# mit-han-lab/qserve

Hardware: AMD Instinct MI355X
Metric: decode tokens/sec/GPU Llama-3-8B W4A8KV4 bs=64 (higher is better)
Workload: dtype int8xint4->int32 (MFMA) + fp16; 1 GPU; Llama-3-8B W4A8 per-channel KV4 decode step, bs=64, context 1024->+512 (BASELINE.json configs[1]); global_batch=64, context_start=1030, parallelism=tp1, hipgraph=True, layers=32, launches_per_layer=8

## Files before the change

qserve_amd/csrc/attention_mfma.hip:

```cpp
#include "attn_host.h"
#include "kv_quant.h"
#include <mutex>
#include <string.h>

namespace {

constexpr int PAGE_TOK = 64;
constexpr int DH = 128;
constexpr int DHB = 64;
constexpr int UT = 32;
constexpr int USB = UT * DHB;
constexpr int NW = attn_plan::DECODE_WAVES_KV4;
constexpr int NWT = NW;
constexpr int QS_ATTNQ_CAP = 4096;
constexpr int QS_ATTNQ_ROW = 4096;
constexpr int SVC = NW - 1;
#ifndef QS_SEQ
#define QS_SEQ(x) asm volatile("" : "+v"(x))
#endif
constexpr int MAXP = 192;

typedef __attribute__((address_space(1))) uint8_t* g_u8;
typedef __attribute__((address_space(1))) uint16_t* g_u16;
__device__ __forceinline__ void wave_quant_store4(_Float16 v0, _Float16 v1, uint8_t* dst_, __half* scale_p_,
                                                  __half* zero_p_, int lane) {
    g_u8 dst = (g_u8)dst_;
    g_u16 scale_p = (g_u16)reinterpret_cast<uint16_t*>(scale_p_), zero_p = (g_u16)reinterpret_cast<uint16_t*>(zero_p_);
    const float mx = wave_max_dpp(fmaxf((float)v0, (float)v1));
    const float mn = wave_min_dpp(fminf((float)v0, (float)v1));
    const QParams p = make_qparams<true>(mn, mx);
    const unsigned u0 = quant_u8(v0, p), u1 = quant_u8(v1, p);
    dst[lane] = (uint8_t)((u0 & 0xFu) | (u1 << 4));
    if (lane == 0) {
        *scale_p = __builtin_bit_cast(uint16_t, p.scale);
        *zero_p = __builtin_bit_cast(uint16_t, p.zero);
    }
}

__device__ __forceinline__ u32 and_or(u32 x, u32 m, u32 c) {
    return (x & m) | c;
}

typedef __attribute__((address_space(3))) const uint8_t* lds_u8;

template <int G, int EXP = 0>
__global__ __launch_bounds__(NWT * 64, 4) void decode_attention_mfma_kernel(
    const _Float16* __restrict__ q, const _Float16* __restrict__ k, const _Float16* __restrict__ v,
    const int64_t* __restrict__ kv_pointers, const int* __restrict__ lengths, _Float16* __restrict__ out,
    int num_heads, int num_kv_heads, int64_t q_stride0, int64_t kv_stride0, int max_blocks, int timestep,
    float rope_base, const float2* __restrict__ rope_tab, int rope_tab_len, int nsplit, float* __restrict__ ws,
    int8_t* __restrict__ qout, __half* __restrict__ qscale, __half* __restrict__ qrowsum, unsigned* __restrict__ qcounters,
    int kflags) {
    constexpr bool PROFILE = (EXP & 64) != 0;
    __shared__ __attribute__((aligned(16))) uint8_t s_kv[2 * NW * 2 * USB];
    __shared__ __attribute__((aligned(16))) _Float16 s_meta[NW][2][4][UT];
    __shared__ __attribute__((aligned(16))) _Float16 s_q[G][DH];
    __shared__ __attribute__((aligned(16))) _Float16 s_qp[16][DH];
    __shared__ __attribute__((aligned(16))) _Float16 s_knew[DH];
    __shared__ __attribute__((aligned(16))) _Float16 s_vnew[DH];
    __shared__ float s_cur[16];
    __shared__ float2 s_qc[16];
    __shared__ float s_m[NW][G], s_l[NW][G];
    __shared__ int s_flag;

    const int tid = threadIdx.x, lane = tid & 63;
    const int wave = __builtin_amdgcn_readfirstlane(tid >> 6);
    const int hkv = blockIdx.x, b = blockIdx.y;
    __shared__ unsigned long long s_stamps[(EXP & 32) ? NWT * 16 : 1];
    auto stamp = [&](int i) {
        if constexpr (EXP & 32) {
            const unsigned long long t = __builtin_amdgcn_s_memtime();
            if (lane == 0) s_stamps[wave * 16 + i] = t;
        }
    };
    if constexpr (EXP & 32) {
        if (lane < 16) s_stamps[wave * 16 + lane] = 0;
    }
    stamp(0);
    if (!(kflags & 2)) {
        const u32 fa = (u32)(uintptr_t)(__attribute__((address_space(3))) void*)(&s_flag);
        if (tid == SVC * 64) asm volatile("ds_write_b32 %0, %1" ::"v"(fa), "v"(0));
        asm volatile("s_waitcnt lgkmcnt(0)\n\ts_barrier");
    }
    const _Float16* qb = q + (size_t)b * q_stride0 + (size_t)hkv * G * DH;
    const _Float16* kb = k + (size_t)b * kv_stride0 + (size_t)hkv * DH;
    const _Float16* vb = v + (size_t)b * kv_stride0 + (size_t)hkv * DH;
    auto uni_ptr = [](const void* x) -> uint64_t {
        return ((uint64_t)(u32)__builtin_amdgcn_readfirstlane((u32)((uint64_t)(uintptr_t)x >> 32)) << 32) |
               (uint64_t)(u32)__builtin_amdgcn_readfirstlane((u32)(uint64_t)(uintptr_t)x);
    };
    const uint64_t qb_s = uni_ptr(qb), kb_s = uni_ptr(kb), vb_s = uni_ptr(vb);
    const int64_t* ktab = kv_pointers + (size_t)b * 2 * max_blocks;
    const int64_t* vtab = ktab + max_blocks;
    const bool spec = (nsplit == 1 || blockIdx.z == 0);
    if (wave == SVC) {
        asm volatile("s_setprio 3");
        if constexpr (!(EXP & 4)) {
            const u32 lane4 = (u32)lane * 4u;
            auto glds4 = [&](uint64_t sb, const _Float16* dst) {
                const u32 ld = __builtin_amdgcn_readfirstlane((u32)(uintptr_t)(__attribute__((address_space(3))) const void*)dst);
                asm volatile("s_mov_b32 m0, %2\n\ts_nop 4\n\tglobal_load_lds_dword %0, %1" ::"v"(lane4), "s"(sb), "s"(ld) : "memory");
            };
#pragma unroll
            for (int h = 0; h < G; ++h) glds4(qb_s + (uint64_t)(h * DH * 2), &s_q[h][0]);
            glds4(kb_s, &s_knew[0]);
            glds4(vb_s, &s_vnew[0]);
        }
        stamp(5);
    }
    int64_t kpage0, vpage0, kpage7, vpage7;
    int len_raw, gen_raw;
    {
        const int p0 = (wave >> 1) < max_blocks ? (wave >> 1) : 0, p7 = ((wave + NW - 1) >> 1) < max_blocks ? ((wave + NW - 1) >> 1) : 0;
        const uint64_t a0 = uni_ptr(ktab + p0), a1 = uni_ptr(vtab + p0), a2 = uni_ptr(ktab + p7), a3 = uni_ptr(vtab + p7);
        const uint64_t a4 = uni_ptr(lengths ? (const void*)(lengths + b) : (const void*)ktab);
        const uint64_t a5 = uni_ptr(qcounters ? (const void*)(qcounters + b) : (const void*)ktab);
        asm volatile("s_load_dwordx2 %0, %6, 0x0\n\ts_load_dwordx2 %1, %7, 0x0\n\ts_load_dwordx2 %2, %8, 0x0\n\t"
                     "s_load_dwordx2 %3, %9, 0x0\n\ts_load_dword %4, %10, 0x0\n\ts_load_dword %5, %11, 0x0\n\ts_waitcnt lgkmcnt(0)"
                     : "=&s"(kpage0), "=&s"(vpage0), "=&s"(kpage7), "=&s"(vpage7), "=&s"(len_raw), "=&s"(gen_raw)
                     : "s"(a0), "s"(a1), "s"(a2), "s"(a3), "s"(a4), "s"(a5)
                     : "memory");
    }
    const int tl = lengths ? len_raw - 1 : timestep;
    if (tl < 0) return;
    stamp(1);
    const float inv_sqrt = 0.08838834764831845f;
    const float qk_scale = inv_sqrt * 1.4426950408889634f;
    constexpr int GP = G <= 4 ? 4 : 8;
    const int li = lane & 15, tg = lane >> 4;
    uint8_t* const s_kw = s_kv + wave * (2 * USB);
    uint8_t* const s_vw = s_kv + (NW + wave) * (2 * USB);

    const int nunits = (tl + UT - 1) >> 5;
    const int z = blockIdx.z;
    const int ups = (nunits + nsplit - 1) / nsplit;
    const int u_begin = z * ups, u_end = min(nunits, u_begin + ups);
    typedef const __attribute__((address_space(1))) void* gptr_t;
    typedef __attribute__((address_space(3))) void* lptr_t;
    auto next_pages = [&](int p, int64_t& kn, int64_t& vn) {
        const uint64_t ka = (uint64_t)(uintptr_t)(ktab + p), va = (uint64_t)(uintptr_t)(vtab + p);
        const uint64_t ks = ((uint64_t)(u32)__builtin_amdgcn_readfirstlane((u32)(ka >> 32)) << 32) |
                            (uint64_t)(u32)__builtin_amdgcn_readfirstlane((u32)ka);
        const uint64_t vs = ((uint64_t)(u32)__builtin_amdgcn_readfirstlane((u32)(va >> 32)) << 32) |
                            (uint64_t)(u32)__builtin_amdgcn_readfirstlane((u32)va);
        asm volatile("s_load_dwordx2 %0, %2, 0x0\n\ts_load_dwordx2 %1, %3, 0x0\n\ts_waitcnt lgkmcnt(0)"
                     : "=&s"(kn), "=&s"(vn) : "s"(ks), "s"(vs) : "memory");
    };
    auto uni64 = [&](int64_t x) -> uint64_t {
        return ((uint64_t)(u32)__builtin_amdgcn_readfirstlane((u32)((uint64_t)x >> 32)) << 32) |
               (uint64_t)(u32)__builtin_amdgcn_readfirstlane((u32)(uint64_t)x);
    };
    auto glds16 = [&](uint64_t sbase, u32 voff, u32 ldst) {
        if constexpr (!(EXP & 1))
            asm volatile("s_mov_b32 m0, %2\n\ts_nop 4\n\tglobal_load_lds_dwordx4 %0, %1 nt" ::"v"(voff), "s"(sbase), "s"(ldst) : "memory");
        else
            asm volatile("s_mov_b32 m0, %2\n\ts_nop 4\n\tglobal_load_lds_dwordx4 %0, %1" ::"v"(voff), "s"(sbase), "s"(ldst) : "memory");
    };
    auto glds4_lower = [&](uint64_t sbase, u32 voff, u32 ldst) {
        uint64_t ex;
        asm volatile("s_mov_b64 %0, exec\n\ts_mov_b32 exec_hi, 0\n\ts_mov_b32 m0, %3\n\ts_nop 4\n\tglobal_load_lds_dword %1, %2\n\ts_mov_b64 exec, %0"
                     : "=&s"(ex) : "v"(voff), "s"(sbase), "s"(ldst) : "memory");
    };
    auto glds4_upper = [&](uint64_t sbase, u32 voff, u32 ldst) {
        uint64_t ex;
        asm volatile("s_mov_b64 %0, exec\n\ts_mov_b32 exec_lo, 0\n\ts_mov_b32 m0, %3\n\ts_nop 4\n\tglobal_load_lds_dword %1, %2\n\ts_mov_b64 exec, %0"
                     : "=&s"(ex) : "v"(voff), "s"(sbase), "s"(ldst) : "memory");
    };
    const u32 meta_lane = (u32)(((lane >> 4) & 1) * num_kv_heads * PAGE_TOK * 2 + (lane & 15) * 4);
    const u32 lane16 = (u32)lane * 16u;
    const u32 lds_k = __builtin_amdgcn_readfirstlane((u32)(uintptr_t)(lptr_t)s_kw);
    const u32 lds_v = __builtin_amdgcn_readfirstlane((u32)(uintptr_t)(lptr_t)s_vw);
    const u32 lds_m = __builtin_amdgcn_readfirstlane((u32)(uintptr_t)(lptr_t)(&s_meta[wave][0][0][0]));
    const u32 meta_off = (u32)(num_kv_heads * PAGE_TOK * DHB + hkv * PAGE_TOK * 2);
    const u32 data_off = (u32)(hkv * PAGE_TOK * DHB);
    auto dma_data = [&](uint64_t base, u32 ldst, int valid_tok) {
        if (valid_tok >= UT) {
            glds16(base, lane16, ldst);
            glds16(base + 1024, lane16, ldst + 1024);
        } else {
            if ((lane >> 2) < valid_tok || lane == 0) glds16(base, lane16, ldst);
            if (16 + (lane >> 2) < valid_tok || lane == 0) glds16(base + 1024, lane16, ldst + 1024);
        }
    };
    auto dma_a = [&](int64_t page, int half, int slot, int valid_tok) {
        const uint64_t pg = uni64(page);
        glds4_lower(pg + (meta_off + (u32)(half * UT * 2)), meta_lane, lds_m + (u32)(slot * (4 * UT * 2)));
        dma_data(pg + (data_off + (u32)(half * USB)), lds_k + (u32)(slot * USB), valid_tok);
    };
    auto dma_b = [&](int64_t page, int half, int slot, int valid_tok) {
        const uint64_t pg = uni64(page);
        glds4_upper(pg + (meta_off + (u32)(half * UT * 2)), meta_lane, lds_m + (u32)(slot * (4 * UT * 2)));
        dma_data(pg + (data_off + (u32)(half * USB)), lds_v + (u32)(slot * USB), valid_tok);
    };
    const int blk = tl >> 6, slot_new = tl & 63;
    const int nu = max(u_end - u_begin, 0);
    const bool svc_free = (nu + NW - 2) / (NW - 1) == (nu + NW - 1) / NW;
    const int PS = svc_free ? NW - 1 : NW;
    const int u_first = u_begin + wave;
    auto unit_of = [&](int i) -> int { return u_first + i * PS; };
    const int cnt = ((!svc_free || wave != SVC) && wave < nu) ? (nu - wave + PS - 1) / PS : 0;
    const bool spec2 = spec && PS == NW - 1;
    const bool use_flag = !(kflags & 2);
    auto first_round = [&](int which) {
        if (cnt > 0) {
            const int u1 = unit_of(1);
            int64_t kfirst = kpage0, vfirst = vpage0, ksecond = kpage7, vsecond = vpage7;
            if ((which & 1) && !spec) next_pages(u_first >> 1, kfirst, vfirst);
            if ((which & 2) && cnt > 1 && !spec2) next_pages(u1 >> 1, ksecond, vsecond);
            if (which & 1) {
                const int vt0 = min(UT, tl - u_first * UT);
                dma_a(kfirst, u_first & 1, 0, vt0);
                stamp(3);
                dma_b(vfirst, u_first & 1, 0, vt0);
            }
            if ((which & 2) && cnt > 1) {
                const int vt1 = min(UT, tl - u1 * UT);
                dma_a(ksecond, u1 & 1, 1, vt1);
                dma_b(vsecond, u1 & 1, 1, vt1);
            }
        }
        if (which & 2) stamp(2);
    };
    auto new_token_work = [&]() {
        if (z == 0) {
            uint8_t* pgk = reinterpret_cast<uint8_t*>(ktab[blk]);
            __half* sck = reinterpret_cast<__half*>(pgk + (size_t)num_kv_heads * PAGE_TOK * DHB);
            wave_quant_store4(s_knew[2 * lane], s_knew[2 * lane + 1], pgk + ((size_t)hkv * PAGE_TOK + slot_new) * DHB,
                              sck + hkv * PAGE_TOK + slot_new, sck + num_kv_heads * PAGE_TOK + hkv * PAGE_TOK + slot_new, lane);
            uint8_t* pgv = reinterpret_cast<uint8_t*>(vtab[blk]);
// ... 70 lines not shown
                so = xor32(xor16(so));
                if (tg == 0) s_qc[li] = make_float2(se + 16.f * so, 1024.f * (se + so));
            }
            if (use_flag) {
                asm volatile("s_waitcnt lgkmcnt(0)" ::: "memory");
                if (lane == 0) *(volatile __attribute__((address_space(3))) int*)(&s_flag) = 1;
            } else {
                asm volatile("s_waitcnt lgkmcnt(0)\n\ts_barrier" ::: "memory");
            }
            asm volatile("s_setprio 0");
            stamp(4);
            if (svc_free) new_token_work();
        } else {
            if (use_flag) {
                asm volatile("s_waitcnt lgkmcnt(0)" ::: "memory");
                if (lane == 0) *(volatile __attribute__((address_space(3))) int*)(&s_flag) = 1;
            } else {
                asm volatile("s_waitcnt lgkmcnt(0)\n\ts_barrier" ::: "memory");
            }
        }
        first_round(3);
    }

    const float2 qc = s_qc[li & (GP - 1)];
    const float qsum = qc.x, nqoff = -qc.y;
    if constexpr (EXP & 32) {
        float probe = nqoff;
        asm volatile("" : "+v"(probe));
        stamp(11);
    }

    u32 c_lo = 0x000F000Fu, c_hi = 0x00F000F0u, c_magic = 0x64006400u;
    asm volatile("" : "+v"(c_lo), "+v"(c_hi), "+v"(c_magic));

    v4f acc[8];
#pragma unroll
    for (int e = 0; e < 8; ++e) acc[e] = (v4f){0.f, 0.f, 0.f, 0.f};
    float m_run = -3.0e38f, l_part = 0.f, corr = 0.f, psum = 0.f;

    constexpr int NS = GP == 4 ? 2 : 4;
    const int tok0 = 16 * (li >> 3) + 4 * tg + (GP == 4 ? 2 * ((li >> 2) & 1) : 0);
    u32 kl0 = (u32)(uintptr_t)(lptr_t)s_kw + (u32)(li * DHB + 16 * tg);
    u32 vl0 = (u32)(uintptr_t)(lptr_t)s_vw + (u32)((4 * tg) * DHB + 4 * li);
    u32 ml0 = (u32)(uintptr_t)(lptr_t)(&s_meta[wave][0][0][0]) + (u32)(2 * tok0);
    asm volatile("" : "+v"(kl0), "+v"(vl0), "+v"(ml0));
    h8 qB[4];
    {
        const lds_u8 ql = (lds_u8)(&s_qp[0][0]) + (li * (DH * 2) + 64 * tg);
#pragma unroll
        for (int w = 0; w < 4; ++w) qB[w] = *(const __attribute__((address_space(3))) h8*)(ql + 16 * w);
    }

    int it = 0;
    int rem = cnt - 1;
    for (int u = u_first; it < cnt; ++it, --rem, u = unit_of(it)) {
        const bool has2 = rem >= 2;
        asm volatile("; QS_LOOP_BEGIN\n\ts_cmp_eq_u32 %0, 0\n\ts_cbranch_scc1 1f\n\ts_waitcnt vmcnt(9)\n\ts_branch 2f\n1:\n\ts_waitcnt vmcnt(3)\n2:"
                     ::"s"(rem) : "memory", "scc");
        if (it < 2) stamp(5 + 2 * it);
        const int slot = it & 1;
        const int valid = min(UT, tl - u * UT);
        const bool full = valid == UT;
        const int u2 = unit_of(it + 2), valid2 = min(UT, tl - u2 * UT);
        int64_t kpage_next = 0, vpage_next = 0;
        if (has2) next_pages(u2 >> 1, kpage_next, vpage_next);
        if constexpr (EXP & 2) {
            if (has2) dma_a(kpage_next, u2 & 1, slot, valid2);
            asm volatile("s_cmp_lt_u32 %0, 2\n\ts_cbranch_scc1 1f\n\ts_waitcnt vmcnt(9)\n\ts_branch 3f\n1:\n\ts_cmp_eq_u32 %0, 0\n\ts_cbranch_scc1 2f\n\t"
                         "s_waitcnt vmcnt(6)\n\ts_branch 3f\n2:\n\ts_waitcnt vmcnt(0)\n3:" ::"s"(rem) : "memory", "scc");
            if (has2) dma_b(vpage_next, u2 & 1, slot, valid2);
            continue;
        }
        const lds_u8 kl = (lds_u8)(kl0 + (u32)(slot * USB));
        const lds_u8 vl = (lds_u8)(vl0 + (u32)(slot * USB));
        const lds_u8 ml = (lds_u8)(ml0 + (u32)(slot * (4 * UT * 2)));
        v4f craw[2];
#pragma unroll
        for (int t = 0; t < 2; ++t) {
            const v4u raw = *(const __attribute__((address_space(3))) v4u*)(kl + 16 * t * DHB);
            v4f c = {nqoff, nqoff, nqoff, nqoff};
#pragma unroll
            for (int w = 0; w < 4; ++w) {
                const u32 x = raw[w], xs = x >> 8;
                const v4u a4 = {and_or(x, c_lo, c_magic), and_or(x, c_hi, c_magic), and_or(xs, c_lo, c_magic),
                                and_or(xs, c_hi, c_magic)};
                c = __builtin_amdgcn_mfma_f32_16x16x32_f16(__builtin_bit_cast(h8, a4), qB[w], c, 0, 0, 0);
            }
            craw[t] = c;
        }
        float sc[NS];
        float m_new;
        {
            float ksf[NS], kzf[NS];
            if constexpr (GP == 4) {
                const h2 ks = *(const __attribute__((address_space(3))) h2*)(ml);
                const h2 kz = *(const __attribute__((address_space(3))) h2*)(ml + UT * 2);
                ksf[0] = (float)ks[0], ksf[1] = (float)ks[1], kzf[0] = (float)kz[0], kzf[1] = (float)kz[1];
            } else {
                const h4 ks = *(const __attribute__((address_space(3))) h4*)(ml);
                const h4 kz = *(const __attribute__((address_space(3))) h4*)(ml + UT * 2);
#pragma unroll
                for (int j = 0; j < 4; ++j) ksf[j] = (float)ks[j], kzf[j] = (float)kz[j];
            }
#pragma unroll
            for (int j = 0; j < NS; ++j) {
                int x;
                if constexpr (GP == 4) {
                    const float c00 = craw[0][j], c02 = craw[0][2 + j], c10 = craw[1][j], c12 = craw[1][2 + j];
                    x = __builtin_bit_cast(int, c00);
                    x = __builtin_amdgcn_update_dpp(x, __builtin_bit_cast(int, c02), 0x114, 0xF, 0x2, false);
                    x = __builtin_amdgcn_update_dpp(x, __builtin_bit_cast(int, c10), 0x118, 0xF, 0x4, false);
                    x = __builtin_amdgcn_update_dpp(x, __builtin_bit_cast(int, c12), 0x11C, 0xF, 0x8, false);
                } else {
                    const float c0 = craw[0][j], c1 = craw[1][j];
                    x = __builtin_amdgcn_update_dpp(__builtin_bit_cast(int, c0), __builtin_bit_cast(int, c1), 0x118, 0xF, 0xC, false);
                }
                sc[j] = (ksf[j] * qk_scale) * (__builtin_bit_cast(float, x) - kzf[j] * qsum);
            }
            if (!full) {
#pragma unroll
                for (int j = 0; j < NS; ++j)
                    if (tok0 + j >= valid) sc[j] = -3.0e38f;
            }
            asm volatile("s_waitcnt lgkmcnt(0)" ::: "memory");
            if (has2) dma_a(kpage_next, u2 & 1, slot, valid2);
            float mx = sc[0];
#pragma unroll
            for (int j = 1; j < NS; ++j) mx = fmaxf(mx, sc[j]);
            if constexpr (GP == 4) asm volatile("s_nop 1\n\tv_max_f32_dpp %0, %0, %0 row_ror:4 row_mask:0xf bank_mask:0xf" : "+v"(mx));
            asm volatile("s_nop 1\n\tv_max_f32_dpp %0, %0, %0 row_ror:8 row_mask:0xf bank_mask:0xf" : "+v"(mx));
            {
                const int xi = __builtin_bit_cast(int, mx);
                const auto r = __builtin_amdgcn_permlane16_swap(xi, xi, false, false);
                mx = fmaxf(__builtin_bit_cast(float, (int)r[0]), __builtin_bit_cast(float, (int)r[1]));
            }
            {
                const int xi = __builtin_bit_cast(int, mx);
                const auto r = __builtin_amdgcn_permlane32_swap(xi, xi, false, false);
                mx = fmaxf(__builtin_bit_cast(float, (int)r[0]), __builtin_bit_cast(float, (int)r[1]));
            }
            m_new = fmaxf(m_run, mx);
            const float alpha = __builtin_amdgcn_exp2f(m_run - m_new);
            m_run = m_new;
            if (__any(alpha != 1.0f)) {
                l_part *= alpha;
                corr *= alpha;
                psum *= alpha;
#pragma unroll
                for (int e = 0; e < 8; ++e) acc[e] *= alpha;
            }
        }
        asm volatile("s_cmp_lt_u32 %0, 2\n\ts_cbranch_scc1 1f\n\ts_waitcnt vmcnt(9)\n\ts_branch 3f\n1:\n\ts_cmp_eq_u32 %0, 0\n\ts_cbranch_scc1 2f\n\t"
                     "s_waitcnt vmcnt(6)\n\ts_branch 3f\n2:\n\ts_waitcnt vmcnt(0)\n3:" ::"s"(rem) : "memory", "scc");
        u32 pbv[4];
        {
            float vsf[NS], vzf[NS];
            if constexpr (GP == 4) {
                const h2 vs = *(const __attribute__((address_space(3))) h2*)(ml + 2 * UT * 2);
                const h2 vz = *(const __attribute__((address_space(3))) h2*)(ml + 3 * UT * 2);
                vsf[0] = (float)vs[0], vsf[1] = (float)vs[1], vzf[0] = (float)vz[0], vzf[1] = (float)vz[1];
            } else {
                const h4 vs = *(const __attribute__((address_space(3))) h4*)(ml + 2 * UT * 2);
                const h4 vz = *(const __attribute__((address_space(3))) h4*)(ml + 3 * UT * 2);
#pragma unroll
                for (int j = 0; j < 4; ++j) vsf[j] = (float)vs[j], vzf[j] = (float)vz[j];
            }
            float pp[NS];
#pragma unroll
            for (int j = 0; j < NS; ++j) {
                const float pe = __builtin_amdgcn_exp2f(sc[j] - m_new);
                l_part += pe;
                float ps = (float)(_Float16)(pe * vsf[j]);
                float pz = ps * vzf[j];
                if (!full && tok0 + j >= valid) {
                    ps = 0.f;
                    pz = 0.f;
                }
                corr += pz;
                psum += ps;
                pp[j] = ps;
            }
            if constexpr (GP == 4) {
                const int pk = (int)pack_h2(pp[0], pp[1]);
                pbv[0] = (u32)pk;
                pbv[1] = (u32)__builtin_amdgcn_update_dpp(0, pk, 0x104, 0xF, 0xF, true);
                pbv[2] = (u32)__builtin_amdgcn_update_dpp(0, pk, 0x108, 0xF, 0xF, true);
                pbv[3] = (u32)__builtin_amdgcn_update_dpp(0, pk, 0x10C, 0xF, 0xF, true);
            } else {
                const int pk0 = (int)pack_h2(pp[0], pp[1]), pk1 = (int)pack_h2(pp[2], pp[3]);
                pbv[0] = (u32)pk0;
                pbv[1] = (u32)pk1;
                pbv[2] = (u32)__builtin_amdgcn_update_dpp(0, pk0, 0x108, 0xF, 0xF, true);
                pbv[3] = (u32)__builtin_amdgcn_update_dpp(0, pk1, 0x108, 0xF, 0xF, true);
            }
        }
        {
            const h8 pB = __builtin_bit_cast(h8, (v4u){pbv[0], pbv[1], pbv[2], pbv[3]});
            u32 raw[8];
#pragma unroll
            for (int jj = 0; jj < 8; ++jj) {
                raw[jj] = *(const __attribute__((address_space(3))) u32*)(vl + (16 * (jj >> 2) + (jj & 3)) * DHB);
            }
#pragma unroll
            for (int bb = 0; bb < 4; ++bb) {
                u32 lo[4], hi[4];
#pragma unroll
                for (int pq = 0; pq < 4; ++pq) {
                    const u32 W = __builtin_amdgcn_perm(raw[2 * pq + 1], raw[2 * pq], 0x0c000c00u | bb | ((4u + bb) << 16));
                    lo[pq] = and_or(W, c_lo, c_magic);
                    hi[pq] = and_or(W, c_hi, c_magic);
                }
                const h8 a_lo = __builtin_bit_cast(h8, (v4u){lo[0], lo[1], lo[2], lo[3]});
                const h8 a_hi = __builtin_bit_cast(h8, (v4u){hi[0], hi[1], hi[2], hi[3]});
                acc[2 * bb] = __builtin_amdgcn_mfma_f32_16x16x32_f16(a_lo, pB, acc[2 * bb], 0, 0, 0);
                acc[2 * bb + 1] = __builtin_amdgcn_mfma_f32_16x16x32_f16(a_hi, pB, acc[2 * bb + 1], 0, 0, 0);
            }
        }
        asm volatile("s_waitcnt lgkmcnt(0) ; QS_LOOP_END" ::: "memory");
        if (it < 2) stamp(6 + 2 * it);
        if (has2) dma_b(vpage_next, u2 & 1, slot, valid2);
    }

    const u32 lid2 = fresh_lane_id();
    const int li2 = lid2 & 15, tg2 = lid2 >> 4, tid2 = wave * 64 + (int)lid2;
    if constexpr (GP == 4) {
        l_part += xor_lane(l_part, lid2, 4);
        corr += xor_lane(corr, lid2, 4);
        psum += xor_lane(psum, lid2, 4);
    }
    l_part += xor_lane(l_part, lid2, 8);
    corr += xor_lane(corr, lid2, 8);
    psum += xor_lane(psum, lid2, 8);
    l_part += xor_lane(l_part, lid2, 16);
    l_part += xor_lane(l_part, lid2, 32);
    corr += xor_lane(corr, lid2, 16);
    corr += xor_lane(corr, lid2, 32);
    psum += xor_lane(psum, lid2, 16);
    psum += xor_lane(psum, lid2, 32);
    if constexpr (!(EXP & 4)) {
        if (wave == SVC && !svc_free) new_token_work();
    }
    asm volatile("s_waitcnt vmcnt(0)" ::: "memory");
    stamp(12);
    __syncthreads();
    stamp(13);
    constexpr int OS = DH + 4;
    float (*s_o)[G][OS] = reinterpret_cast<float (*)[G][OS]>(&s_kv[0]);
    static_assert(sizeof(float) * NW * G * OS <= sizeof(s_kv), "merge area must fit the page buffers");
    if (li2 < G) {
#pragma unroll
        for (int e = 0; e < 8; ++e)
#pragma unroll
            for (int r = 0; r < 4; ++r)
                s_o[wave][li2][8 * (4 * tg2 + r) + e] = ((e & 1) ? acc[e][r] * 0.0625f : acc[e][r]) - (corr + ((e & 1) ? 64.f : 1024.f) * psum);
        if (tg2 == 0) {
            s_m[wave][li2] = m_run;
            s_l[wave][li2] = l_part;
        }
    }
    __syncthreads();
    stamp(14);
    for (int o = tid2; o < G * DH; o += NWT * 64) {
        const int h = o / DH, d = o % DH;
        float M = z == 0 ? s_cur[h] : -3.0e38f;
#pragma unroll
        for (int w = 0; w < NW; ++w) M = fmaxf(M, s_m[w][h]);
        const float pc = z == 0 ? __builtin_amdgcn_exp2f(s_cur[h] - M) : 0.f;
        float num = pc * (float)((EXP & 4) ? vb[d] : s_vnew[d]), den = pc;
#pragma unroll
        for (int w = 0; w < NW; ++w) {
            const float f = __builtin_amdgcn_exp2f(s_m[w][h] - M);
            num += f * s_o[w][h][d];
            den += f * s_l[w][h];
        }
        if (nsplit == 1) {
            const _Float16 res = (_Float16)(num / (den + 1.e-6f));
            if (qout) reinterpret_cast<_Float16*>(&s_meta[0][0][0])[o] = res;
            else out[((size_t)b * num_heads + (size_t)hkv * G + h) * DH + d] = res;
        } else {
            float* pw = ws + ((((size_t)b * num_kv_heads + hkv) * nsplit + z) * G + h) * (DH + 2);
            pw[d] = num;
            if (d == 0) {
                pw[DH] = M * 0.6931471805599453f;
                pw[DH + 1] = den;
            }
        }
    }
    if (nsplit == 1 && qout) {
        __syncthreads();
        const int hidden = num_heads * DH;
        const unsigned tag = (unsigned)gen_raw + 1u;
        if (tid2 < G * 16) {
            const v4u x = reinterpret_cast<const v4u*>(&s_meta[0][0][0])[tid2];
            *reinterpret_cast<v4u*>(out + ((size_t)b * num_heads + (size_t)hkv * G) * DH + tid2 * 8) = x;
        }
        v2u* const xrow = reinterpret_cast<v2u*>(qcounters + QS_ATTNQ_CAP) + (size_t)b * (QS_ATTNQ_ROW / 2);
        const int own_lo = (num_kv_heads - 1) * G * DH;
        if ((G == 4 || G == 8) && !(kflags & 1024)) {
            float* const sm = reinterpret_cast<float*>(&s_kv[0]);
            v4u* const gran = reinterpret_cast<v4u*>(xrow);
            if (wave == 0) {
                const int ln = (int)lid2;
                float amax = 0.f, s0 = 0.f, s1 = 0.f;
                {
                    const h8 vv = __builtin_bit_cast(h8, reinterpret_cast<const v4u*>(&s_meta[0][0][0])[ln]);
#pragma unroll
                    for (int j = 0; j < 8; ++j) {
                        const float f = (float)vv[j];
                        s0 += f;
                        QS_SEQ(s0);
                        amax = fmaxf(amax, fabsf(f));
                    }
                }
                if (G == 8) {
                    const h8 vv = __builtin_bit_cast(h8, reinterpret_cast<const v4u*>(&s_meta[0][0][0])[64 + ln]);
#pragma unroll
                    for (int j = 0; j < 8; ++j) {
                        const float f = (float)vv[j];
                        s1 += f;
                        QS_SEQ(s1);
                        amax = fmaxf(amax, fabsf(f));
                    }
                }
                amax = wave_max(amax);
                s0 = wave_sum(s0);
                if (G == 8) s1 = wave_sum(s1);
                v4u mine = {__builtin_bit_cast(u32, amax), __builtin_bit_cast(u32, s0), __builtin_bit_cast(u32, s1), tag};
                if (ln == 0 && !((kflags & 64) && b == 0 && hkv == 0) && !(kflags & 512)) {
                    v4u* const dst = gran + hkv;
                    asm volatile("global_store_dwordx4 %0, %1, off sc0 sc1" ::"v"(dst), "v"(mine) : "memory");
                }
                const __amdgpu_buffer_rsrc_t grs = __builtin_amdgcn_make_buffer_rsrc(gran, 0, num_kv_heads * 16, 0x00020000);
                const bool peer = ln < num_kv_heads && ln != hkv;
                const u32 goff = ln < num_kv_heads ? (u32)ln * 16u : 0xFFFFFF00u;
                const int spin_cap = (kflags & 256) ? 1 : (kflags & 64) ? 4096 : QS_SPIN_CAP;
                int polls = 0;
                v4u g;
                for (;;) {
                    g = __builtin_amdgcn_raw_buffer_load_b128(grs, goff, 0, 17);
                    if (!__builtin_amdgcn_ballot_w64(peer && g.w != tag)) break;
                    if (++polls >= spin_cap) {
                        if (ln == 0 && !(kflags & 256))
                            atomicOr(qcounters + QS_ATTNQ_CAP + (size_t)QS_ATTNQ_CAP * QS_ATTNQ_ROW, QS_ERR_ATTN_HANDOVER);
                        break;
                    }
                    __builtin_amdgcn_s_sleep(1);
                }
                if (ln == hkv) g = mine;
                const u32 gx = g.x, gy = g.y, gz = g.z;
                float am = ln < num_kv_heads ? __builtin_bit_cast(float, gx) : 0.f;
                am = wave_max(am);
                float bs;
                if (G == 4) {
                    bs = ln < num_kv_heads ? __builtin_bit_cast(float, gy) : -0.0f;
                } else {
                    const int src = (ln >> 1) < num_kv_heads ? (ln >> 1) : 0;
                    const int yv = __builtin_amdgcn_ds_bpermute(4 * src, (int)gy), zv = __builtin_amdgcn_ds_bpermute(4 * src, (int)gz);
                    bs = (ln >> 1) < num_kv_heads ? __builtin_bit_cast(float, (ln & 1) ? zv : yv) : -0.0f;
                }
                const float tot = wave_sum(bs);
                if (ln == 0) {
                    sm[0] = am;
                    sm[1] = tot;
                }
            }
            __syncthreads();
            const float r = sm[0];
            if (tid2 < G * 16) {
                const h8 vv = __builtin_bit_cast(h8, reinterpret_cast<const v4u*>(&s_meta[0][0][0])[tid2]);
                float f[8];
#pragma unroll
                for (int j = 0; j < 8; ++j) f[j] = (float)vv[j];
                qs_store_q8(qout + (size_t)b * hidden + (size_t)hkv * G * DH + tid2 * 8, f, 127.0f / r);
            }
            if (hkv == num_kv_heads - 1 && tid2 == 0) {
                qscale[b] = __float2half_rn(r / 127.0f);
                if (qrowsum) qrowsum[b] = __float2half_rn(sm[1]);
                qcounters[b] = tag;
            }
        } else if (hkv != num_kv_heads - 1) {
            for (int e = tid2; e < G * DH / 2 && !((kflags & 64) && b == 0 && hkv == 0) && !(kflags & 512); e += NWT * 64) {
                v2u gr;
                gr.x = reinterpret_cast<const u32*>(&s_meta[0][0][0])[e];
                gr.y = tag;
                v2u* const dst = xrow + (size_t)hkv * (G * DH / 2) + e;
                asm volatile("global_store_dwordx2 %0, %1, off sc0 sc1" ::"v"(dst), "v"(gr) : "memory");
            }
        } else {
            const __amdgpu_buffer_rsrc_t xrs = __builtin_amdgcn_make_buffer_rsrc(xrow, 0, QS_ATTNQ_ROW * 4, 0x00020000);
            v4u raw[2] = {{0, 0, 0, 0}, {0, 0, 0, 0}};
            if (tid2 < 256) {
                const int i0 = tid2 * 8, i1 = (256 + tid2) * 8;
                const bool p0 = i0 < own_lo, p1 = i1 < own_lo;
                const u32 o0 = p0 ? (u32)i0 * 4u : 0xFFFFFF00u, o1 = p1 ? (u32)i1 * 4u : 0xFFFFFF00u;
                const int spin_cap = (kflags & 256) ? 1 : (kflags & 64) ? 4096 : QS_SPIN_CAP;
                int polls = 0;
                for (;;) {
                    const v4u g00 = __builtin_amdgcn_raw_buffer_load_b128(xrs, o0, 0, 17);
                    const v4u g01 = __builtin_amdgcn_raw_buffer_load_b128(xrs, o0, 16, 17);
                    const v4u g10 = __builtin_amdgcn_raw_buffer_load_b128(xrs, o1, 0, 17);
                    const v4u g11 = __builtin_amdgcn_raw_buffer_load_b128(xrs, o1, 16, 17);
                    const int m0 = (g00.y != tag) | (g00.w != tag) | (g01.y != tag) | (g01.w != tag);
                    const int m1 = (g10.y != tag) | (g10.w != tag) | (g11.y != tag) | (g11.w != tag);
                    raw[0] = (v4u){g00.x, g00.z, g01.x, g01.z};
                    raw[1] = (v4u){g10.x, g10.z, g11.x, g11.z};
                    if (!__builtin_amdgcn_ballot_w64((p0 && m0) || (p1 && m1))) break;
                    if (++polls >= spin_cap) {
                        if ((tid2 & 63) == 0 && !(kflags & 256))
                            atomicOr(qcounters + QS_ATTNQ_CAP + (size_t)QS_ATTNQ_CAP * QS_ATTNQ_ROW, QS_ERR_ATTN_HANDOVER);
                        break;
                    }
                    __builtin_amdgcn_s_sleep(1);
                }
                if (!p0 && i0 < hidden) raw[0] = reinterpret_cast<const v4u*>(&s_meta[0][0][0])[(i0 - own_lo) >> 3];
                if (!p1 && i1 < hidden) raw[1] = reinterpret_cast<const v4u*>(&s_meta[0][0][0])[(i1 - own_lo) >> 3];
            }
            float* const sm = reinterpret_cast<float*>(&s_kv[0]);
            float amax = 0.f, sum[2] = {0.f, 0.f};
            if (tid2 < 256) {
#pragma unroll
                for (int c = 0; c < 2; ++c) {
                    const int i = (c * 256 + tid2) * 8;
                    if (i < hidden) {
                        const h8 vv = __builtin_bit_cast(h8, raw[c]);
#pragma unroll
                        for (int j = 0; j < 8; ++j) {
                            const float f = (float)vv[j];
                            sum[c] += f;
                            QS_SEQ(sum[c]);
                            amax = fmaxf(amax, fabsf(f));
                        }
                    }
                }
                amax = wave_max(amax);
                if (qrowsum) {
                    sum[0] = wave_sum(sum[0]);
                    sum[1] = wave_sum(sum[1]);
                }
                if ((tid2 & 63) == 0) {
                    sm[tid2 >> 6] = amax;
                    sm[4 + (tid2 >> 6)] = sum[0];
                    sm[8 + (tid2 >> 6)] = sum[1];
                }
            }
            __syncthreads();
            if (tid2 < 256) {
                float r = sm[0];
#pragma unroll
                for (int w = 1; w < 4; ++w) r = fmaxf(r, sm[w]);
                float s2 = 0.f;
                if (qrowsum && tid2 < 64) s2 = wave_sum(tid2 < (hidden + 511) / 512 ? sm[4 + tid2] : -0.0f);
                if (tid2 == 0) {
                    qscale[b] = __float2half_rn(r / 127.0f);
                    if (qrowsum) qrowsum[b] = __float2half_rn(s2);
                    qcounters[b] = tag;
                }
                const float mul = 127.0f / r;
#pragma unroll
                for (int c = 0; c < 2; ++c) {
                    const int i = (c * 256 + tid2) * 8;
                    if (i < hidden) {
                        const h8 vv = __builtin_bit_cast(h8, raw[c]);
                        float f[8];
#pragma unroll
                        for (int j = 0; j < 8; ++j) f[j] = (float)vv[j];
                        qs_store_q8(qout + (size_t)b * hidden + i, f, mul);
                    }
                }
            }
        }
    }
    stamp(15);
    if constexpr (EXP & 32) {
        if (lane < 16)
            reinterpret_cast<unsigned long long*>(ws)[(((size_t)b * gridDim.x + hkv) * NWT + wave) * 16 + lane] = s_stamps[wave * 16 + lane];
    }
}

__global__ __launch_bounds__(DH) void decode_attention_merge_kernel(const float* __restrict__ ws, _Float16* __restrict__ out,
                                                                    int num_heads, int num_kv_heads, int G, int nsplit) {
    const int b = blockIdx.y, hq = blockIdx.x, d = threadIdx.x;
    const int hkv = hq / G, h = hq % G;
    const float* base = ws + (((size_t)b * num_kv_heads + hkv) * nsplit * G + h) * (DH + 2);
    const size_t zs = (size_t)G * (DH + 2);
    float M = -3.0e38f;
    for (int zz = 0; zz < nsplit; ++zz) M = fmaxf(M, base[zz * zs + DH]);
    float num = 0.f, den = 0.f;
    for (int zz = 0; zz < nsplit; ++zz) {
        const float f = __expf(base[zz * zs + DH] - M);
        num += f * base[zz * zs + d];
        den += f * base[zz * zs + DH + 1];
    }
    out[((size_t)b * num_heads + hq) * DH + d] = (_Float16)(num / (den + 1.e-6f));
}

__global__ void rope_table_kernel(float2* tab, int max_pos, float base) {
    const int i = blockIdx.x * blockDim.x + threadIdx.x;
    if (i >= max_pos * 64) return;
    const RopeCS cs = rope_coef_any(i & 63, i >> 6, base, DH, tab);
    tab[i] = make_float2(cs.c, cs.s);
}

struct RopeTable {
    float2* tab = nullptr;
    int len = 0;
    float base = 0.f;
};
constexpr int ROPE_SLOTS = 8;
RopeTable g_rope[16][ROPE_SLOTS];
std::mutex g_rope_mutex;

constexpr int ROPE_PROFILES = 8, ROPE_PROFILE_TABLES = 12;
struct RopeProfile {
    float denom[64];
    float mscale;
    RopeTable tabs[16][ROPE_PROFILE_TABLES];
};
RopeProfile g_profile[ROPE_PROFILES];
int g_profiles = 0;

int profile_of_key(float key) {
    const float idf = -key - 1.0f;
    const int id = idf >= 0.f && idf < (float)ROPE_PROFILES ? (int)idf : -1;
    return id >= 0 && id < g_profiles && (float)id == idf ? id : -1;
}
const RopeTable* longest_profile_table(const RopeProfile& p, int dev) {
    const RopeTable* best = nullptr;
    for (const RopeTable& r : p.tabs[dev])
        if (r.tab && (!best || r.len > best->len)) best = &r;
    return best;
}
const RopeTable* build_profile_table(int id, int dev, int rows, hipStream_t st) {
    RopeProfile& p = g_profile[id];
    RopeTable* slot = nullptr;
    for (RopeTable& r : p.tabs[dev])
        if (!r.tab && !slot) slot = &r;
    if (!slot) return nullptr;
    float2 head[ROPE_PROFILE_HEAD];
    for (int i = 0; i < ROPE_PROFILE_HEAD; ++i) head[i] = make_float2(p.denom[i], p.mscale);
    void* mem = nullptr;
    if (hipMalloc(&mem, ((size_t)rows * 64 + ROPE_PROFILE_HEAD) * sizeof(float2)) != hipSuccess) {
        (void)hipGetLastError();
        return nullptr;
    }
    float2* tab = reinterpret_cast<float2*>(mem) + ROPE_PROFILE_HEAD;
    bool ok = hipMemcpyAsync(mem, head, sizeof(head), hipMemcpyHostToDevice, st) == hipSuccess;
    if (ok) hipLaunchKernelGGL(rope_table_kernel, dim3((rows * 64 + 255) / 256), dim3(256), 0, st, tab, rows, -(float)(id + 1));
    if (!ok || hipGetLastError() != hipSuccess || hipStreamSynchronize(st) != hipSuccess) {
        (void)hipGetLastError();
        (void)hipFree(mem);
        return nullptr;
    }
    slot->len = rows, slot->base = -(float)(id + 1), slot->tab = tab;
    return slot;
}
bool capturing(hipStream_t st) {
    hipStreamCaptureStatus cs = hipStreamCaptureStatusNone;
    if (hipStreamIsCapturing(st, &cs) != hipSuccess) {
        (void)hipGetLastError();
        return true;
    }
    return cs != hipStreamCaptureStatusNone;
}
const float2* profile_table(float key, int max_pos, int dev, hipStream_t st, int* len_out) {
    const int id = profile_of_key(key);
    if (id < 0) {
        qs_set_error("rotary base %g: a negative base is the key of a RoPE profile, and no profile with this key is registered", (double)key);
        return nullptr;
    }
    const RopeTable* t = longest_profile_table(g_profile[id], dev);
    if (!t) {
        qs_set_error("rotary base %g: RoPE profile %d is not registered on device %d (qs_rope_profile_register on that device)", (double)key,
                     id, dev);
        return nullptr;
    }
    if (t->len < max_pos && !capturing(st)) {
        const RopeTable* longer = build_profile_table(id, dev, max_pos, st);
        if (longer) t = longer;
    }
    *len_out = t->len;
    return t->tab;
}

}

extern "C" int qs_rope_profile_register(const float* denom, int pairs, float mscale, int table_positions, float* key_out) {
    QS_REQUIRE(denom && key_out, "rope_profile_register: null pointer");
    QS_REQUIRE(pairs == 64, "rope_profile_register: pairs=%d, only 64 (head_dim 128) is supported", pairs);
    QS_REQUIRE(table_positions > 0 && table_positions <= 32768, "rope_profile_register: table_positions=%d not in 1 .. 32768", table_positions);
    QS_REQUIRE(mscale > 0.f && mscale < INFINITY, "rope_profile_register: mscale must be positive and finite");
    for (int i = 0; i < 64; ++i) QS_REQUIRE(denom[i] > 0.f && denom[i] < INFINITY, "rope_profile_register: denom[%d] must be positive and finite", i);
    std::lock_guard<std::mutex> lock(g_rope_mutex);
    int dev = 0;
    if (hipGetDevice(&dev) != hipSuccess || dev < 0 || dev >= 16) {
        (void)hipGetLastError();
        qs_set_error("rope_profile_register: no current device");
        return QS_EINVAL;
    }
    hipStream_t st = nullptr;
    if (capturing(st)) {
        qs_set_error("rope_profile_register: called inside a stream capture - register before capturing (the table is built eagerly)");
        return QS_EINVAL;
    }
    int id = -1;
    for (int i = 0; i < g_profiles && id < 0; ++i)
        if (!memcmp(g_profile[i].denom, denom, sizeof(float) * 64) && !memcmp(&g_profile[i].mscale, &mscale, sizeof(float))) id = i;
    const bool fresh = id < 0;
    if (fresh) {
        if (g_profiles == ROPE_PROFILES) {
            qs_set_error("rope_profile_register: all %d RoPE profiles of this process are taken", ROPE_PROFILES);
            return QS_EINVAL;
        }
        id = g_profiles;
        memcpy(g_profile[id].denom, denom, sizeof(float) * 64);
        g_profile[id].mscale = mscale;
        ++g_profiles;
    }
    const RopeTable* t = longest_profile_table(g_profile[id], dev);
    if ((!t || t->len < table_positions) && !build_profile_table(id, dev, table_positions, st) && !t) {
        if (fresh) --g_profiles;
        qs_set_error("rope_profile_register: the table of %d positions could not be built on device %d (out of memory, or a stream "
                     "capture in progress: register before capturing)", table_positions, dev);
        return QS_EINVAL;
    }
    *key_out = -(float)(id + 1);
    return QS_OK;
}

// ... 54 lines not shown
        if (!r.tab && !slot) slot = &r;
    }
    if (!slot) return nullptr;
    hipStreamCaptureStatus cs = hipStreamCaptureStatusNone;
    if (hipStreamIsCapturing(st, &cs) != hipSuccess || cs != hipStreamCaptureStatusNone) {
        (void)hipGetLastError();
        return nullptr;
    }
    void* p = nullptr;
    if (hipMalloc(&p, (size_t)max_pos * 64 * sizeof(float2)) != hipSuccess) {
        (void)hipGetLastError();
        return nullptr;
    }
    hipLaunchKernelGGL(rope_table_kernel, dim3((max_pos * 64 + 255) / 256), dim3(256), 0, st, reinterpret_cast<float2*>(p),
                       max_pos, base);
    if (hipStreamSynchronize(st) != hipSuccess) {
        (void)hipGetLastError();
        (void)hipFree(p);
        return nullptr;
    }
    slot->len = max_pos;
    slot->base = base;
    slot->tab = reinterpret_cast<float2*>(p);
    *len_out = slot->len;
    return slot->tab;
}

namespace {
constexpr size_t SPLIT_WS_BYTES = (size_t)32 << 20;
struct SplitWs {
    float* p = nullptr;
};
SplitWs g_ws[16][QS_MAX_STREAM_SLOTS];
}
void qs_launch_attention_merge(const float* ws, _Float16* out, int H, int Hkv, int G, int nsplit, int batch,
                               hipStream_t st) {
    hipLaunchKernelGGL(decode_attention_merge_kernel, dim3(H, batch), dim3(DH), 0, st, ws, out, H, Hkv, G, nsplit);
}
float* qs_split_workspace(size_t bytes, hipStream_t st) {
    int dev = 0;
    if (bytes > SPLIT_WS_BYTES || hipGetDevice(&dev) != hipSuccess || dev < 0 || dev >= 16) return nullptr;
    SplitWs& w = g_ws[dev][qs_scratch_slot(st)];
    if (w.p) return w.p;
    hipStreamCaptureStatus cs = hipStreamCaptureStatusNone;
    if (hipStreamIsCapturing(st, &cs) != hipSuccess || cs != hipStreamCaptureStatusNone) {
        (void)hipGetLastError();
        return nullptr;
    }
    void* p = nullptr;
    if (hipMalloc(&p, SPLIT_WS_BYTES) != hipSuccess) {
        (void)hipGetLastError();
        return nullptr;
    }
    w.p = reinterpret_cast<float*>(p);
    return w.p;
}
size_t qs_split_workspace_capacity() { return SPLIT_WS_BYTES; }

extern "C" int qs_debug_copy_split_workspace(void* dst, size_t bytes) {
    int dev = 0;
    if (hipGetDevice(&dev) != hipSuccess || dev < 0 || dev >= 16 || !g_ws[dev][0].p || bytes > SPLIT_WS_BYTES) return QS_EINVAL;
    return (int)hipMemcpy(dst, g_ws[dev][0].p, bytes, hipMemcpyDeviceToDevice);
}

namespace {
unsigned* g_qcounters[16][QS_MAX_STREAM_SLOTS];
}
unsigned* qs_attn_quant_counters(hipStream_t st, int batch) {
    int dev = 0;
    if (batch > QS_ATTNQ_CAP || hipGetDevice(&dev) != hipSuccess || dev < 0 || dev >= 16) return nullptr;
    unsigned*& slot_p = g_qcounters[dev][qs_scratch_slot(st)];
    if (slot_p) return slot_p;
    hipStreamCaptureStatus cs = hipStreamCaptureStatusNone;
    if (hipStreamIsCapturing(st, &cs) != hipSuccess || cs != hipStreamCaptureStatusNone) {
        (void)hipGetLastError();
        return nullptr;
    }
    void* p = nullptr;
    const size_t bytes = (size_t)QS_ATTNQ_CAP * 4 + (size_t)QS_ATTNQ_CAP * QS_ATTNQ_ROW * 4 + 64;
    if (hipMalloc(&p, bytes) != hipSuccess || hipMemset(p, 0, bytes) != hipSuccess || hipDeviceSynchronize() != hipSuccess) {
        (void)hipGetLastError();
        return nullptr;
    }
    slot_p = reinterpret_cast<unsigned*>(p);
    return slot_p;
}

unsigned* qs_attn_error_word(int slot) {
    int dev = 0;
    if (hipGetDevice(&dev) != hipSuccess || dev < 0 || dev >= 16 || slot < 0 || slot >= QS_MAX_STREAM_SLOTS || !g_qcounters[dev][slot])
        return nullptr;
    return g_qcounters[dev][slot] + QS_ATTNQ_CAP + (size_t)QS_ATTNQ_CAP * QS_ATTNQ_ROW;
}
bool qs_attn_scratch_prealloc(hipStream_t st) {
    const bool a = qs_split_workspace(1, st) != nullptr;
    const bool b = qs_attn_quant_counters(st, 1) != nullptr;
    return a && b;
}
int qs_attn_reset_handoff() {
    int dev = 0;
    if (hipGetDevice(&dev) != hipSuccess || dev < 0 || dev >= 16) return QS_OK;
    const size_t bytes = (size_t)QS_ATTNQ_CAP * 4 + (size_t)QS_ATTNQ_CAP * QS_ATTNQ_ROW * 4 + 64;
    for (int slot = 0; slot < QS_MAX_STREAM_SLOTS; ++slot) {
        if (!g_qcounters[dev][slot]) continue;
        hipError_t e = hipMemset(g_qcounters[dev][slot], 0, bytes);
        if (e == hipSuccess) e = hipDeviceSynchronize();
        if (e != hipSuccess) {
            qs_set_error("qs_device_reset (attention): %s", hipGetErrorString(e));
            return (int)e;
        }
    }
    return QS_OK;
}

int qs_launch_decode_mfma(const DecodeArgs& a, const attn_plan::AttnPlan& plan) {
    QS_DECODE_LOCALS(a);
    const QsAttnQuant* const quant = a.quant;
    bool* const fused = a.fused;
    int kflags = plan.kflags, exp_flags = plan.exp_flags;
    int tab_len = 0;
    const float2* tab = qs_rope_table(base, max_pos, st, &tab_len);
    if (base < 0.f && !tab) return QS_EINVAL;
    const int blocks = (int)(grid.x * grid.y);
    const size_t per_split = attn_plan::decode_split_bytes(blocks, G);
    int nsplit = plan.nsplit > 1 ? attn_plan::fit_splits(plan.nsplit, per_split, qs_split_workspace_capacity(), attn_plan::NO_SPLIT_CAP) : 1;
    float* ws = nsplit > 1 ? qs_split_workspace(per_split * nsplit, st) : nullptr;
    if (!ws) nsplit = 1;
    grid.z = nsplit;
    int8_t* qout = nullptr;
    __half *qscale = nullptr, *qsum = nullptr;
    unsigned* qcnt = nullptr;
    const bool sum_order_ok = !(quant && qs_get_row_sum_order() && quant->qsum);
    if (quant && sum_order_ok && nsplit == 1 && H * DH <= 4096 && (qcnt = qs_attn_quant_counters(st, (int)grid.y))) {
        qout = quant->qout;
        qscale = reinterpret_cast<__half*>(quant->qscale);
        qsum = reinterpret_cast<__half*>(quant->qsum);
        *fused = true;
        if (g_inject_fault & 2) kflags |= 64, g_inject_fault &= ~2;
    }
#define QS_LAUNCH_GP(KERNEL)                                                                                                      \
    hipLaunchKernelGGL((KERNEL), grid, dim3(NWT * 64), 0, st, q, k, v, kvp, len, out, H, Hkv, qs, kvs, mb, timestep, base, tab, tab_len, \
                       nsplit, ws, qout, qscale, qsum, qcnt, kflags)
#define QS_LAUNCH_G(GG)                                                \
    if (base < 0.f) QS_LAUNCH_GP((decode_attention_mfma_kernel<GG, 64>));  \
    else QS_LAUNCH_GP(decode_attention_mfma_kernel<GG>)
#define QS_LAUNCH_EXP(E)                                                                                              \
    case E:                                                                                                            \
        hipLaunchKernelGGL((decode_attention_mfma_kernel<4, E>), grid, dim3(NWT * 64), 0, st, q, k, v, kvp, len, out, H,  \
                           Hkv, qs, kvs, mb, timestep, base, tab, tab_len, nsplit, ws, qout, qscale, qsum, qcnt, kflags); \
        return qs_launch_status("single_query_attention")
#ifdef QS_TIMING
    if (const char* e = getenv("QS_ATTN_KFLAGS")) kflags = atoi(e);
    if (exp_flags & 32) {
        ws = qs_split_workspace((size_t)blocks * NWT * 16 * 8, st);
        if (!ws) exp_flags = 0;
    }
    if (G == 4 && exp_flags > 0 && nsplit == 1) {
        switch (exp_flags) {
            QS_LAUNCH_EXP(1);
            QS_LAUNCH_EXP(2);
            QS_LAUNCH_EXP(4);
            QS_LAUNCH_EXP(6);
            QS_LAUNCH_EXP(32);
            default: break;
        }
    }
#endif
    switch (G) {
        case 1: QS_LAUNCH_G(1); break;
        case 2: QS_LAUNCH_G(2); break;
        case 3: QS_LAUNCH_G(3); break;
        case 4: QS_LAUNCH_G(4); break;
        case 5: QS_LAUNCH_G(5); break;
        case 6: QS_LAUNCH_G(6); break;
        case 7: QS_LAUNCH_G(7); break;
        case 8: QS_LAUNCH_G(8); break;
        default:
            qs_set_error("single_query_attention: num_heads/num_kv_heads = %d not in 1..8", G);
            return QS_ENOSUP;
    }
#undef QS_LAUNCH_G
#undef QS_LAUNCH_GP
    if (nsplit > 1)
        hipLaunchKernelGGL(decode_attention_merge_kernel, dim3(H, grid.y), dim3(DH), 0, st, ws, out, H, Hkv, G, nsplit);
    return qs_launch_status("single_query_attention");
}
```

Baseline: 22710 tokens/s.

## Drop barrier before attention merge and fuse output quantization into wave zero

Each wave now writes its partial output into its own K ring slot with swizzled vector stores, so the barrier before the merge writes is removed and one LDS barrier stays. The merge loop handles two elements per thread with paired loads and stores. The fused int8 output quantization is done entirely by wave 0 after the cross-head gather, while wave 1 writes the fp16 output, removing a block-wide sync and an LDS round trip. Timing stamps are extended from 16 to 24 slots for profiling. The risk is a race if any wave still reads its own ring when another wave's data is consumed, and wave 0 now carries more serial work.

```diff
diff --git a/qserve_amd/csrc/attention_mfma.hip b/qserve_amd/csrc/attention_mfma.hip
--- a/qserve_amd/csrc/attention_mfma.hip
+++ b/qserve_amd/csrc/attention_mfma.hip
@@ -66,15 +66,15 @@
     const int tid = threadIdx.x, lane = tid & 63;
     const int wave = __builtin_amdgcn_readfirstlane(tid >> 6);
     const int hkv = blockIdx.x, b = blockIdx.y;
-    __shared__ unsigned long long s_stamps[(EXP & 32) ? NWT * 16 : 1];
+    __shared__ unsigned long long s_stamps[(EXP & 32) ? NWT * 24 : 1];
     auto stamp = [&](int i) {
         if constexpr (EXP & 32) {
             const unsigned long long t = __builtin_amdgcn_s_memtime();
-            if (lane == 0) s_stamps[wave * 16 + i] = t;
+            if (lane == 0) s_stamps[wave * 24 + i] = t;
         }
     };
     if constexpr (EXP & 32) {
-        if (lane < 16) s_stamps[wave * 16 + lane] = 0;
+        if (lane < 24) s_stamps[wave * 24 + lane] = 0;
     }
     stamp(0);
     if (!(kflags & 2)) {
@@ -451,6 +451,7 @@
         }
         asm volatile("s_cmp_lt_u32 %0, 2\n\ts_cbranch_scc1 1f\n\ts_waitcnt vmcnt(9)\n\ts_branch 3f\n1:\n\ts_cmp_eq_u32 %0, 0\n\ts_cbranch_scc1 2f\n\t"
                      "s_waitcnt vmcnt(6)\n\ts_branch 3f\n2:\n\ts_waitcnt vmcnt(0)\n3:" ::"s"(rem) : "memory", "scc");
+        if (rem == 0) stamp(16);
         u32 pbv[4];
         {
             float vsf[NS], vzf[NS];
@@ -541,68 +542,88 @@
     }
     asm volatile("s_waitcnt vmcnt(0)" ::: "memory");
     stamp(12);
-    __syncthreads();
-    stamp(13);
-    constexpr int OS = DH + 4;
-    float (*s_o)[G][OS] = reinterpret_cast<float (*)[G][OS]>(&s_kv[0]);
-    static_assert(sizeof(float) * NW * G * OS <= sizeof(s_kv), "merge area must fit the page buffers");
+    static_assert(sizeof(float) * G * DH <= 2 * USB, "a wave's partial must fit its own K ring");
     if (li2 < G) {
-#pragma unroll
-        for (int e = 0; e < 8; ++e)
-#pragma unroll
-            for (int r = 0; r < 4; ++r)
-                s_o[wave][li2][8 * (4 * tg2 + r) + e] = ((e & 1) ? acc[e][r] * 0.0625f : acc[e][r]) - (corr + ((e & 1) ? 64.f : 1024.f) * psum);
+        float* const s_ow = reinterpret_cast<float*>(s_kw) + li2 * DH;
+#pragma unroll
+        for (int r = 0; r < 4; ++r)
+#pragma unroll
+            for (int e0 = 0; e0 < 8; e0 += 4) {
+                v4f x;
+#pragma unroll
+                for (int j = 0; j < 4; ++j) {
+                    const int e = e0 + j;
+                    x[j] = ((e & 1) ? acc[e][r] * 0.0625f : acc[e][r]) - (corr + ((e & 1) ? 64.f : 1024.f) * psum);
+                }
+                *reinterpret_cast<v4f*>(s_ow + ((8 * (4 * tg2 + r) + e0) ^ (4 * li2))) = x;
+            }
         if (tg2 == 0) {
             s_m[wave][li2] = m_run;
             s_l[wave][li2] = l_part;
         }
     }
-    __syncthreads();
+    stamp(17);
+    asm volatile("s_waitcnt lgkmcnt(0)\n\ts_barrier" ::: "memory");
     stamp(14);
-    for (int o = tid2; o < G * DH; o += NWT * 64) {
+    for (int o = 2 * tid2; o < G * DH; o += 2 * NWT * 64) {
         const int h = o / DH, d = o % DH;
         float M = z == 0 ? s_cur[h] : -3.0e38f;
 #pragma unroll
         for (int w = 0; w < NW; ++w) M = fmaxf(M, s_m[w][h]);
         const float pc = z == 0 ? __builtin_amdgcn_exp2f(s_cur[h] - M) : 0.f;
-        float num = pc * (float)((EXP & 4) ? vb[d] : s_vnew[d]), den = pc;
+        h2 vn;
+        if constexpr (EXP & 4) vn = (h2){vb[d], vb[d + 1]};
+        else vn = *reinterpret_cast<const h2*>(&s_vnew[d]);
+        float num0 = pc * (float)vn[0], num1 = pc * (float)vn[1], den = pc;
 #pragma unroll
         for (int w = 0; w < NW; ++w) {
             const float f = __builtin_amdgcn_exp2f(s_m[w][h] - M);
-            num += f * s_o[w][h][d];
+            const float2 so = *reinterpret_cast<const float2*>(reinterpret_cast<const float*>(s_kv + w * (2 * USB)) + h * DH + (d ^ (4 * h)));
+            num0 += f * so.x;
+            num1 += f * so.y;
             den += f * s_l[w][h];
         }
         if (nsplit == 1) {
-            const _Float16 res = (_Float16)(num / (den + 1.e-6f));
-            if (qout) reinterpret_cast<_Float16*>(&s_meta[0][0][0])[o] = res;
-            else out[((size_t)b * num_heads + (size_t)hkv * G + h) * DH + d] = res;
+            const h2 res = {(_Float16)(num0 / (den + 1.e-6f)), (_Float16)(num1 / (den + 1.e-6f))};
+            if (qout) *reinterpret_cast<h2*>(reinterpret_cast<_Float16*>(&s_meta[0][0][0]) + o) = res;
+            else *reinterpret_cast<h2*>(out + ((size_t)b * num_heads + (size_t)hkv * G + h) * DH + d) = res;
         } else {
             float* pw = ws + ((((size_t)b * num_kv_heads + hkv) * nsplit + z) * G + h) * (DH + 2);
-            pw[d] = num;
+            *reinterpret_cast<float2*>(pw + d) = make_float2(num0, num1);
             if (d == 0) {
                 pw[DH] = M * 0.6931471805599453f;
                 pw[DH + 1] = den;
             }
         }
     }
+    stamp(18);
     if (nsplit == 1 && qout) {
         __syncthreads();
+        stamp(19);
         const int hidden = num_heads * DH;
         const unsigned tag = (unsigned)gen_raw + 1u;
-        if (tid2 < G * 16) {
-            const v4u x = reinterpret_cast<const v4u*>(&s_meta[0][0][0])[tid2];
-            *reinterpret_cast<v4u*>(out + ((size_t)b * num_heads + (size_t)hkv * G) * DH + tid2 * 8) = x;
+        const bool gather = (G == 4 || G == 8) && !(kflags & 1024);
+        v4u* const orow = reinterpret_cast<v4u*>(out + ((size_t)b * num_heads + (size_t)hkv * G) * DH);
+        if (!gather && tid2 < G * 16) {
+            orow[tid2] = reinterpret_cast<const v4u*>(&s_meta[0][0][0])[tid2];
         }
         v2u* const xrow = reinterpret_cast<v2u*>(qcounters + QS_ATTNQ_CAP) + (size_t)b * (QS_ATTNQ_ROW / 2);
         const int own_lo = (num_kv_heads - 1) * G * DH;
-        if ((G == 4 || G == 8) && !(kflags & 1024)) {
-            float* const sm = reinterpret_cast<float*>(&s_kv[0]);
+        if (gather) {
             v4u* const gran = reinterpret_cast<v4u*>(xrow);
+            if (wave == 1) {
+                const int ln = (int)lid2;
+                orow[ln] = reinterpret_cast<const v4u*>(&s_meta[0][0][0])[ln];
+                if (G == 8) orow[64 + ln] = reinterpret_cast<const v4u*>(&s_meta[0][0][0])[64 + ln];
+            }
             if (wave == 0) {
                 const int ln = (int)lid2;
+                const v4u x0 = reinterpret_cast<const v4u*>(&s_meta[0][0][0])[ln];
+                v4u x1 = {0, 0, 0, 0};
+                if (G == 8) x1 = reinterpret_cast<const v4u*>(&s_meta[0][0][0])[64 + ln];
                 float amax = 0.f, s0 = 0.f, s1 = 0.f;
                 {
-                    const h8 vv = __builtin_bit_cast(h8, reinterpret_cast<const v4u*>(&s_meta[0][0][0])[ln]);
+                    const h8 vv = __builtin_bit_cast(h8, x0);
 #pragma unroll
                     for (int j = 0; j < 8; ++j) {
                         const float f = (float)vv[j];
@@ -612,7 +633,7 @@
                     }
                 }
                 if (G == 8) {
-                    const h8 vv = __builtin_bit_cast(h8, reinterpret_cast<const v4u*>(&s_meta[0][0][0])[64 + ln]);
+                    const h8 vv = __builtin_bit_cast(h8, x1);
 #pragma unroll
                     for (int j = 0; j < 8; ++j) {
                         const float f = (float)vv[j];
@@ -629,6 +650,7 @@
                     v4u* const dst = gran + hkv;
                     asm volatile("global_store_dwordx4 %0, %1, off sc0 sc1" ::"v"(dst), "v"(mine) : "memory");
                 }
+                stamp(20);
                 const __amdgpu_buffer_rsrc_t grs = __builtin_amdgcn_make_buffer_rsrc(gran, 0, num_kv_heads * 16, 0x00020000);
                 const bool peer = ln < num_kv_heads && ln != hkv;
                 const u32 goff = ln < num_kv_heads ? (u32)ln * 16u : 0xFFFFFF00u;
@@ -645,6 +667,7 @@
                     }
                     __builtin_amdgcn_s_sleep(1);
                 }
+                stamp(21);
                 if (ln == hkv) g = mine;
                 const u32 gx = g.x, gy = g.y, gz = g.z;
                 float am = ln < num_kv_heads ? __builtin_bit_cast(float, gx) : 0.f;
@@ -658,24 +681,21 @@
                     bs = (ln >> 1) < num_kv_heads ? __builtin_bit_cast(float, (ln & 1) ? zv : yv) : -0.0f;
                 }
                 const float tot = wave_sum(bs);
-                if (ln == 0) {
-                    sm[0] = am;
-                    sm[1] = tot;
-                }
-            }
-            __syncthreads();
-            const float r = sm[0];
-            if (tid2 < G * 16) {
-                const h8 vv = __builtin_bit_cast(h8, reinterpret_cast<const v4u*>(&s_meta[0][0][0])[tid2]);
-                float f[8];
-#pragma unroll
-                for (int j = 0; j < 8; ++j) f[j] = (float)vv[j];
-                qs_store_q8(qout + (size_t)b * hidden + (size_t)hkv * G * DH + tid2 * 8, f, 127.0f / r);
-            }
-            if (hkv == num_kv_heads - 1 && tid2 == 0) {
-                qscale[b] = __float2half_rn(r / 127.0f);
-                if (qrowsum) qrowsum[b] = __float2half_rn(sm[1]);
-                qcounters[b] = tag;
+                const float r = am;
+#pragma unroll
+                for (int c = 0; c < G / 4; ++c) {
+                    const h8 vv = __builtin_bit_cast(h8, c ? x1 : x0);
+                    float f[8];
+#pragma unroll
+                    for (int j = 0; j < 8; ++j) f[j] = (float)vv[j];
+                    qs_store_q8(qout + (size_t)b * hidden + (size_t)hkv * G * DH + (c * 64 + ln) * 8, f, 127.0f / r);
+                }
+                if (hkv == num_kv_heads - 1 && ln == 0) {
+                    qscale[b] = __float2half_rn(r / 127.0f);
+                    if (qrowsum) qrowsum[b] = __float2half_rn(tot);
+                    qcounters[b] = tag;
+                }
+                stamp(22);
             }
         } else if (hkv != num_kv_heads - 1) {
             for (int e = tid2; e < G * DH / 2 && !((kflags & 64) && b == 0 && hkv == 0) && !(kflags & 512); e += NWT * 64) {
@@ -771,8 +791,8 @@
     }
     stamp(15);
     if constexpr (EXP & 32) {
-        if (lane < 16)
-            reinterpret_cast<unsigned long long*>(ws)[(((size_t)b * gridDim.x + hkv) * NWT + wave) * 16 + lane] = s_stamps[wave * 16 + lane];
+        if (lane < 24)
+            reinterpret_cast<unsigned long long*>(ws)[(((size_t)b * gridDim.x + hkv) * NWT + wave) * 24 + lane] = s_stamps[wave * 24 + lane];
     }
 }
 
@@ -1133,7 +1153,7 @@
 #ifdef QS_TIMING
     if (const char* e = getenv("QS_ATTN_KFLAGS")) kflags = atoi(e);
     if (exp_flags & 32) {
-        ws = qs_split_workspace((size_t)blocks * NWT * 16 * 8, st);
+        ws = qs_split_workspace((size_t)blocks * NWT * 24 * 8, st);
         if (!ws) exp_flags = 0;
     }
     if (G == 4 && exp_flags > 0 && nsplit == 1) {
```

After: 22850 tokens/s (median of 6 runs). No clear change (+0.6%).
